# JacobYuan7/DIN-Group-Activity-Recognition-Benchmark

Measured on AMD Instinct MI355X. Metric: clips/sec (fwd+bwd), Volleyball DIN stage-2, BxTx12 actors, higher is better.
Workload: dtype bf16; 1 GPU; Volleyball stage-2 DIN, inv3, T=3, ST_kernel=(3,3), N=12, 720x1280, bf16; global_batch=32, clips_per_gpu=32, frames=3, parallelism=dp1, includes=fwd + cross-entropy + bwd + fused Adam (lr 0), launch_mode=eager launches, bn_mode=running statistics (set_bn_eval)

## Files before the change

din-group-activity-recognition-benchmark_amd/_lib.py:

```python
from __future__ import annotations

import ctypes as C
import os
import re
import subprocess
from typing import Dict, List

_HERE = os.path.dirname(os.path.abspath(__file__))
LIB_PATH = os.environ.get("DIN_LIB_PATH") or os.path.join(_HERE, "libdin_hip.so")
CSRC_DIR = os.path.join(_HERE, "csrc")
HEADER_PATH = os.path.join(os.path.dirname(_HERE), "include", "din_hip.h")

DIN_F32, DIN_BF16 = 0, 1
DIN_F32_BF16X3 = 2


def storage_dtype(dt: int) -> int:
    return DIN_F32 if dt == DIN_F32_BF16X3 else dt
ABI_VERSION = 9
CONV_BIAS, CONV_RELU, CONV_ACCUM, CONV_MASK = 1, 2, 4, 8


class DinError(RuntimeError):
    pass
# ... 34 lines not shown

SIGNATURES: Dict[str, tuple] = {
    "din_abi_version": (_I, []),
    "din_last_error_string": (C.c_char_p, []),
    "din_set_option": (_I, [C.c_char_p, C.c_char_p]),
    "din_get_option": (_I, [C.c_char_p, C.c_char_p, _I]),
    "din_build_arch": (C.c_char_p, []),
    "din_prep_images_f32": (_I, [_P, _P, _L, _P]),
    "din_prep_images_nhwc": (_I, [_P, _I, _P, _I, _I, _I, _I, _I, _P]),
    "din_conv_packed_elems": (_L, [_CD, _I]),
    "din_conv_pack_weights": (_I, [_CD, _P, _P, _P, _I, _P]),
    "din_conv_pack_desc": (_I, [_CD, _P, _P, _P, _I, C.POINTER(PackDesc)]),
    "din_conv_pack_multi": (_I, [_P, _P, _P, _I, _I, _P]),
    "din_conv_kernel_tile": (_I, [_CD, _I, C.POINTER(C.c_int32), C.POINTER(C.c_int32)]),
    "din_conv_kernel_variant": (_I, [_CD, _I, C.POINTER(C.c_int32)]),
    "din_conv_kernel_names": (_I, [_CD, _I, _I, _I, _I, C.c_char_p, _I]),
    "din_conv_workspace_bytes": (_L, [_CD, _I]),
    "din_conv_accepts_u8": (_I, [_P]),
    "din_conv_fwd": (_I, [_CD, _P, _P, _P, _P, _I, _P, _L, _P]),
    "din_conv_fwd2": (_I, [_CD, _P, _P, _P, _P, _P, _I, _I, _I, _I, _I, _P, _L, _P]),
    "din_conv_fwd2_kernel_names": (_I, [_CD, _I, _I, _I, _I, _I, C.c_char_p, _I]),
    "din_conv_dgrad": (_I, [_CD, _P, _P, _P, _P, _I, _I, _I, _P, _L, _P]),
    "din_conv1x1_dgrad_multi": (_I, [_I, C.POINTER(ConvSrc), _I, _I, _I, _I, _I, _I, _I, _P, _P, _I, _I, _I, _P]),
    "din_conv1x1_dgrad_multi_kernel_names": (_I, [_I, C.POINTER(ConvSrc), _I, _I, _I, _I, _I, _I, _I, _I, _I, _I, C.c_char_p, _I]),
    "din_conv_dgrad_x_fused": (_I, [_CD]),
    "din_conv_dgrad_x": (_I, [_CD, _P, _P, _P, _P, _I, _I, _I, C.POINTER(ConvSrc), _P, _L, _P]),
    "din_conv_dgrad_x_kernel_names": (_I, [_CD, C.POINTER(ConvSrc), _I, _I, _I, C.c_char_p, _I]),
    "din_conv1x1_wgrad_multi_workspace": (_L, [_I, C.POINTER(ConvWSrc), _I, _L, _I]),
    "din_conv1x1_wgrad_multi": (_I, [_I, C.POINTER(ConvWSrc), _I, _L, _I, _I, _I, _P, _I, _P, _L, _P]),
    "din_conv_wgrad_group_key": (_I, [_CD]),
    "din_conv_wgrad_group_workspace": (_L, [_I, C.POINTER(ConvWgradItem)]),
    "din_conv_wgrad_group": (_I, [_I, C.POINTER(ConvWgradItem), _P, _L, _P]),
    "din_conv_wgrad": (_I, [_CD, _P, _P, _P, _P, _P, _P, _P, _I, _P, _L, _P]),
    "din_colsum": (_I, [_P, _I, _L, _I, _I, _I, _P, _P]),
    "din_bn_fold": (_I, [_P, _P, _P, _P, _F, _P, _P, _I, _P]),
    "din_bn_fold_bwd": (_I, [_P, _P, _P, _P, _F, _P, _P, _I, _P]),
    "din_bn_fold_multi": (_I, [_P, _P, _I, _I, _F, _P, _P, _P]),
    "din_bn_fold_bwd_multi": (_I, [_P, _P, _I, _I, _F, _P, _P, _P, _P, _P]),
    "din_bn_stats": (_I, [_P, _I, _L, _I, _I, _I, _P, _P, _P]),
    "din_bn_parts": (_I, [_L]),
    "din_bn_workspace": (_L, [_L, _I]),
    "din_bn_reduce": (_I, [_P, _I, _I, _P]),
    "din_bn_finalize": (_I, [_P, _I, _L, _I, _P, _P, _F, _F, _P, _P, _P, _P, _P, _P, _P, _P]),
    "din_bn_apply": (_I, [_P, _I, _L, _I, _I, _I, _P, _P, _I, _P, _I, _I, _P]),
    "din_bn_bwd_stats": (_I, [_P, _I, _I, _P, _I, _I, _I, _L, _I, _P, _P, _P, _P]),
    "din_bn_bwd_apply": (_I, [_P, _I, _I, _P, _I, _I, _I, _L, _I, _P, _P, _P, _P, _P, _I, _I, _P, _P, _P]),
    "din_maxpool_fwd": (_I, [_PD, _P, _P, _P, _P]),
    "din_maxpool_bwd": (_I, [_PD, _P, _P, _P, _P, _I, _I, _P]),
    "din_avgpool_fwd": (_I, [_PD, _P, _P, _P, _I, _P]),
    "din_avgpool_bwd": (_I, [_PD, _P, _P, _P, _I, _P]),
    "din_bilinear_fwd": (_I, [_PD, _P, _P, _P]),
    "din_bilinear_bwd": (_I, [_PD, _P, _P, _P, _I, _P]),
    "din_pool_kernel_name": (_I, [_PD, _I, _I, _I, _I, C.c_char_p, _I]),
    "din_roi_align_fwd": (_I, [_P, _I, _I, _I, _I, _I, _I, _I, _I, _P, _P, _I, _I, _P, _I, _I, _P, _P]),
    "din_roi_align_bwd": (_I, [_P, _I, _I, _I, _I, _P, _P, _I, _I, _P, _P]),
    "din_roi_crop_grad_transpose": (_I, [_P, _I, _I, _I, _P, _P]),
    "din_roi_align_bwd_nhwc": (_I, [_P, _I, _I, _I, _I, _I, _I, _I, _I, _I, _P, _P, _I, _I, _P, _I, _I, _P, _I, _P]),
    "din_grad_cast_mask": (_I, [_P, _P, _P, _I, _L, _I, _I, _I, _I, _I, _I, _P]),
    "din_boxes_frame_index": (_I, [_P, _I, _I, _P]),
    "din_layernorm_fwd": (_I, [_P, _P, _P, _P, _F, _P, _P, _L, _L, _I, _F, _U64, _P, _P]),
    "din_layernorm_bwd": (_I, [_P, _P, _P, _P, _P, _P, _P, _P, _P, _L, _L, _I, _F, _U64, _P, _P]),
    "din_counter_add": (_I, [_P, _U64, _P]),
    "din_walk_fwd": (_I, [_P, _P, _I, _I, _I, _I, _I, _I, _I, _I, _I, _I, _P, _P, _P, _P, _P, _P, _P]),
    "din_walk_bwd": (_I, [_P, _P, _I, _P, _P, _I, _I, _I, _I, _I, _I, _I, _I, _I, _P, _P, _P, _P, _P, _P]),
    "din_head_fwd": (_I, [_P, _P, _P, _P, _I, _I, _I, _I, _I, _P, _P, _P]),
    "din_head_bwd": (_I, [_P, _P, _P, _P, _I, _I, _I, _I, _I, _P, _P, _P, _P]),
# ... 108 lines not shown
```

din-group-activity-recognition-benchmark_amd/csrc/conv_wgrad.h:

```cpp
#pragma once
#include "din_common.h"
#include <string>

namespace din_wgrad {

struct WgradK {
    const void* in; const void* g; float* partial; float* dbias;
    int NB, H, W, Cin, ldi, cioff;
    int OH, OW, Cout, ldo, cooff;
    int kh, kw, sh, sw, ph, pw, dh, dw;
    int cin_pad, kcols, kcols_pad, cout_pad;
    int M, n_co_tiles, n_k_tiles, slices, m_per_slice;
    int probe;
    const unsigned char* u8;
    int atomic;
    int pace_base;
    float* direct;
    int* pace;
};

constexpr int WGRAD_GROUP_MAX = 16;
struct WgradGroupK { WgradK k[WGRAD_GROUP_MAX]; int first[WGRAD_GROUP_MAX + 1]; int n; };

struct Wg1x1K {
// ... 7 lines not shown

__device__ __forceinline__ void lds_dma16(uint32_t lds_addr, __amdgpu_buffer_rsrc_t rs, int voff, int soff) {
    asm volatile("s_mov_b32 m0, %0\n\ts_nop 0\n\tbuffer_load_dwordx4 %1, %2, %3 offen lds"
                 :: "s"(lds_addr), "v"(voff), "s"(rs), "s"(soff) : "memory", "m0");
}

enum WgradFamily {
    WGRAD_F32,
    WGRAD_F32X3,
    WGRAD_BF16_TAIL,
    WGRAD_BF16,
    WGRAD_RING,
    WGRAD_PIPE,
    WGRAD_STEM,
    WGRAD_HALO
};
struct PipeInst { int bco, bk; bool wide; int wn; };
struct StemInst { int cpp, bn, st; bool u8; int nw, th, ring; };
struct HaloInst { int cpp, bnt, kh, kw, th; };
struct WgradChoice {
    WgradFamily family;
    int bco, bk;
    PipeInst pipe; StemInst stem; HaloInst halo;
    dim3 grid, block; size_t lds;
    bool bias_fused;
    int atomic;
    int group_key;
    int cin_pad, kcols, kcols_pad, cout_pad, n_co_tiles, n_k_tiles, slices, m_per_slice;
    int64_t ws_bytes;
};
WgradChoice plan_wgrad(const din_conv_desc* d, bool split = false);
void wgrad_tile_code(const WgradChoice& c, int32_t* bm, int32_t* bn);
void append_wgrad_names(const din_conv_desc* d, const WgradChoice& c, std::string& out);

int launch_wgrad_pipe(const WgradK& k, const PipeInst& inst, dim3 grid, dim3 block, size_t lds, hipStream_t st);
int launch_wgrad_pipe_group(const WgradGroupK& g, int bco, bool wide, hipStream_t st);
size_t wgrad_pipe_lds_bytes(int bco, int bk);
bool wgrad_halo_shape(int cin, int cout, int kh, int kw, HaloInst* inst);
size_t wgrad_halo_lds_bytes(const HaloInst& inst);
int launch_wgrad_halo(const WgradK& k, const HaloInst& inst, dim3 grid, dim3 block, size_t lds, hipStream_t st);
bool plan_wgrad_1x1_multi(int nsrc, const int* couts, int cin, Wg1x1K* k);
int launch_wgrad_1x1_multi(const Wg1x1K& k, int nwg, hipStream_t st);

}
```

din-group-activity-recognition-benchmark_amd/csrc/conv_wgrad.hip:

```cpp
#include "din_common.h"
#include "conv_wgrad.h"
#include "conv_shared.h"
#include <atomic>
#include <string>

using din_wgrad::WgradK;
using din_wgrad::WgradChoice;
using din_wgrad::lds_dma16;
using din_conv::check_desc;

namespace {

constexpr int WG_TILE = 128;

template <bool SPLIT>
__device__ __forceinline__ void conv_wgrad_f32_body(const WgradK& p) {
    constexpr int PK = 16;
    constexpr int RS = WG_TILE + 16;
    __shared__ float Gs[2][PK][RS];
    __shared__ float Xs[2][PK][RS];
    const int tid = threadIdx.x, lane = tid & 63, wid = tid >> 6;
    const int wm = wid >> 1, wn = wid & 1;
    int bid, slice_;
    xcd_block(bid, slice_);
// ... 1244 lines not shown
    } else if (v2) {
        w.family = WGRAD_BF16;
        w.lds = 2 * 64 * ((size_t)(w.bco * 2) + (WG_TILE * 2));
    } else {
        w.family = WGRAD_BF16_TAIL;
        w.lds = 2 * 2 * 32 * (WG_TILE * 2 + 32);
    }
    w.bias_fused = w.family != WGRAD_F32 && w.family != WGRAD_F32X3 && w.family != WGRAD_BF16_TAIL;
    return w;
}

void wgrad_tile_code(const WgradChoice& c, int32_t* bm, int32_t* bn) {
    switch (c.family) {
    case WGRAD_HALO: *bm = 3; *bn = c.bco; break;
    case WGRAD_STEM: *bm = 0; *bn = c.bco; break;
    case WGRAD_PIPE: *bm = c.bco; *bn = 2000 + c.bk; break;
    case WGRAD_RING: *bm = c.bco; *bn = 1000 + c.bk; break;
    default: *bm = c.bco; *bn = WG_TILE; break;
    }
}

void append_wgrad_names(const din_conv_desc* d, const WgradChoice& c, std::string& out) {
    out += wgrad_kernel_name(c); out += '\n';
    out += "conv_wgrad_reduce_kernel\n";
    if (!c.bias_fused) {
        const int unr = colsum_unroll(d->dtype, d->cout, d->ldo, d->cooff);
        const char* T = d->dtype == DIN_F32 ? "float" : "unsigned short";
        char s[64];
        if (unr) snprintf(s, sizeof s, "colsum_vec_kernel<%s, %d>\n", T, unr); else snprintf(s, sizeof s, "colsum_kernel<%s>\n", T);
        out += s;
    }
}

}

extern "C" {

int din_conv_wgrad(const din_conv_desc* d, const void* in, const void* dout, float* dw, float* dbias, const float* scale,
                   const float* w, float* wdot, int accumulate, void* workspace, int64_t workspace_bytes, void* stream) {
    const SplitDesc sd(d);
    if (int e = check_desc(d)) return e;
    DIN_REQUIRE(in && dout && dw, "conv_wgrad: null pointer");
    DIN_REQUIRE(!wdot || w, "conv_wgrad: wdot needs w");
    DIN_REQUIRE(!d->in_u8 || din_conv_accepts_u8(d), "conv_wgrad: in_u8 on a layer din_conv_accepts_u8() rejects");
    hipStream_t st = as_stream(stream);
    const bool prezeroed = (accumulate & 2) != 0;
    accumulate &= 1;
    const WgradChoice c = din_wgrad::plan_wgrad(d, sd.split);
    if (workspace_bytes < c.ws_bytes || !workspace)
        DIN_FAIL(DIN_E_WORKSPACE, "conv_wgrad: workspace %lld < %lld bytes", (long long)workspace_bytes, (long long)c.ws_bytes);
    DIN_REQUIRE(d->dtype == DIN_F32 || (d->ldo % 8 == 0 && d->cooff % 8 == 0), "conv_wgrad: bf16 dout stride/offset must be multiples of 8");
    WgradK k{};
    fill_wgrad_k(k, d, c, in, dout, workspace);
#ifdef DIN_EXPERIMENTS
    { const char* pv = DIN_OPT("DIN_WGRAD_PROBE"); k.probe = pv ? atoi(pv) : 0; }
#else
    k.probe = 0;
#endif
    if (dbias && c.bias_fused) {
        if (!prezeroed && hipMemsetAsync(dbias, 0, sizeof(float) * d->cout, st) != hipSuccess) DIN_FAIL(DIN_E_LAUNCH, "conv_wgrad: memset");
        k.dbias = dbias;
    }
    if (c.family == din_wgrad::WGRAD_PIPE) {
        k.atomic = c.atomic;
        if (c.atomic && hipMemsetAsync(k.partial, 0, sizeof(float) * (size_t)c.cout_pad * c.kcols_pad, st) != hipSuccess)
            DIN_FAIL(DIN_E_LAUNCH, "conv_wgrad: memset");
// ... 236 lines not shown
```

din-group-activity-recognition-benchmark_amd/nhwc.py:

```python
from __future__ import annotations

import ctypes as C
from dataclasses import dataclass, field
from typing import Dict, List, NamedTuple, Optional, Sequence, Tuple

import torch

from . import _lib as L


def _ptr(t: Optional[torch.Tensor]):
    return C.c_void_p(t.data_ptr()) if t is not None else None


def _stream():
    return C.c_void_p(torch.cuda.current_stream().cuda_stream)


def torch_dtype(dt: int):
    return torch.float32 if L.storage_dtype(dt) == L.DIN_F32 else torch.bfloat16


def din_dtype(t: torch.Tensor) -> int:
    if t.dtype == torch.float32:
        return L.DIN_F32
    if t.dtype == torch.bfloat16:
        return L.DIN_BF16
    raise L.DinError(f"unsupported storage dtype {t.dtype}")


def require_gpu(*tensors: torch.Tensor) -> None:
    for t in tensors:
        if t is None:
            continue
        if not t.is_cuda:
            raise L.DinError("din_amd ops run only on MI355X device tensors (no CPU fallback); got a CPU tensor")
        if not t.is_contiguous():
            raise L.DinError("din_amd ops need contiguous tensors")


import contextlib as _contextlib
LAUNCH_TIMER = None
TIMING_ACTIVE = lambda: LAUNCH_TIMER is not None


def _timed(kind, d, name=""):
    return LAUNCH_TIMER(kind, d, name) if LAUNCH_TIMER is not None else _contextlib.nullcontext()


GRAD_HOOK = None
GRAD_TAP = None
GRAD_BUFFER = None
GRAD_ASSIGN = None


def _dw_buffer(w: torch.Tensor) -> torch.Tensor:
    if GRAD_BUFFER is not None:
        buf = GRAD_BUFFER(w)
        if buf is not None:
            return buf
    return torch.empty_like(w)
FUSE_1X1_DGRAD = None
FUSE_FWD_SIBLINGS = None
FUSE_WGRAD_SIBLINGS = None
FUSE_WGRAD_1X1 = None
FUSE_DGRAD_X = None
GROUP_WGRAD = None
GROUP_WGRAD_MAX = 12
GROUP_WGRAD_MB = 768
_SWITCHES = {"FUSE_1X1_DGRAD": ("DIN_FUSE_1X1", True), "FUSE_FWD_SIBLINGS": ("DIN_FUSE_FWD", True), "FUSE_WGRAD_SIBLINGS": ("DIN_FUSE_WGRAD", True),
             "FUSE_WGRAD_1X1": ("DIN_FUSE_WGRAD_1X1", True), "FUSE_DGRAD_X": ("DIN_FUSE_DGRAD_X", True), "GROUP_WGRAD": ("DIN_GROUP_WGRAD", True), "WGRAD_SIDE_STREAM": ("DIN_WGRAD_STREAM", False)}


def switch(attr: str) -> bool:
    v = globals()[attr]
    if v is not None:
        return bool(v)
    name, default = _SWITCHES[attr]
    return L.host_flag(name, default)



_WS: Dict[Tuple[int, str], torch.Tensor] = {}


_SIDE: Dict[int, "torch.cuda.Stream"] = {}
WGRAD_SIDE_STREAM = None


def side_stream(device) -> "torch.cuda.Stream":
    key = device.index if device.index is not None else torch.cuda.current_device()
    if key not in _SIDE:
        _SIDE[key] = torch.cuda.Stream(device=device)
    return _SIDE[key]


def workspace(nbytes: int, device, tag: str = "") -> Tuple[Optional[torch.Tensor], int]:
    if nbytes <= 0:
        return None, 0
    key = (device.index if device.index is not None else torch.cuda.current_device(), tag)
    ws = _WS.get(key)
    if ws is None or ws.numel() < nbytes:
        ws = torch.empty(int(nbytes * 1.25) + 1024, dtype=torch.uint8, device=device)
        _WS[key] = ws
# ... 415 lines not shown
            aux.append((amax,))
        elif op.kind in ("avgpool", "bilinear"):
            d = _pool_desc(g, op, nb, dt)
            if op.kind == "avgpool":
                L.check(lib.din_avgpool_fwd(C.byref(d), _ptr(src), _ptr(dst), None, 0, st), "avgpool_fwd")
            else:
                L.check(lib.din_bilinear_fwd(C.byref(d), _ptr(src), _ptr(dst), st), "bilinear_fwd")
            aux.append(())
        else:
            raise L.DinError("unknown op " + op.kind)
    return bufs, aux


ViewKey = Tuple[int, int, int]


@dataclass
class BackwardPlan:
    offsets: List[int]
    bn_index: Dict[int, int]
    bn_train: bool
    side: bool
    u8: bool
    dgrad_groups: Dict[ViewKey, List[int]]
    member_of: Dict[int, ViewKey]
    x_host: Dict[int, int]
    siblings: Dict[int, Tuple[int, ...]]
    multi_w: Dict[ViewKey, Tuple[List[Tuple[int, ...]], int]]
    group_on: bool
    group_max: int
    group_bytes: int
    partitioned: set
    first_writer: Dict[int, int]


def _partitioned(readers: List[Tuple[int, int]], writers: Sequence[Tuple[int, int]]) -> bool:
    for (a0, ac), (b0, _bc) in zip(readers, readers[1:]):
        if b0 < a0 + ac:
            return False
    for lo, c in writers:
        hi = lo + c
        for c0, cc in readers:
            if c0 <= lo < c0 + cc:
                lo = min(hi, c0 + cc)
        if lo < hi:
            return False
    return True


def wgrad_queue_full(layers: int, held_bytes: int, max_layers: int, max_bytes: int) -> bool:
    return layers >= max_layers or held_bytes >= max_bytes


def plan_backward(g: Graph, nb: int, dt: int, bn_train: bool, side_ok: bool, u8: bool) -> BackwardPlan:
    lib = L.load()
    offsets, bn_index, pos = [], {}, 0
    readers: Dict[int, set] = {}
    writers: Dict[int, list] = {}
    first_writer: Dict[int, int] = {}
    for oi, op in enumerate(g.ops):
        if op.kind == "conv":
            offsets.append(pos)
            if op.bn:
                bn_index[oi] = len(bn_index)
            pos += 5 if op.bn else (2 if op.bias else 1)
        else:
# ... 29 lines not shown
        for grp in g.fwd_groups:
            mem = tuple(i for i in grp[1:] if g.ops[i].pooled is None)
            if len(mem) >= 2 and g.ops[mem[-1]].bn:
                siblings[mem[-1]] = mem
    multi_w: Dict[ViewKey, Tuple[List[Tuple[int, ...]], int]] = {}
    if switch("FUSE_WGRAD_1X1") and bn_index and not bn_train and not side and bf16:
        pair_of = {i: mem for mem in siblings.values() for i in mem}
        for key, members in groups.items():
            if not all(g.ops[i].bn for i in members):
                continue
            plan, seen = [], set()
            for i in members:
                if i in seen:
                    continue
                mem = pair_of.get(i, (i,))
                if not all(j in members for j in mem):
                    mem = (i,)
                plan.append(tuple(mem))
                seen.update(mem)
            probe = (L.ConvWSrc * len(plan))()
            for j, mem in enumerate(plan):
                o = g.ops[mem[0]]
                probe[j].cout = sum(g.ops[i].dst.c for i in mem)
                probe[j].ldo, probe[j].cooff = (o.dst.c, 0) if o.pooled is not None else (g.tensors[o.dst.tid].c, o.dst.coff)
            o0 = g.ops[members[0]]
            ts0 = g.tensors[o0.src.tid]
            need = lib.din_conv1x1_wgrad_multi_workspace(len(plan), probe, dt, nb * ts0.h * ts0.w, o0.src.c) if 2 <= len(plan) <= 4 else 0
            if need > 0:
                multi_w[key] = (plan, need)
    group_on = switch("GROUP_WGRAD") and bf16 and not side
    group_max = max(2, min(16, int(L.get_option("DIN_GROUP_WGRAD_MAX") or GROUP_WGRAD_MAX))) if group_on else 0
    group_bytes = int(L.get_option("DIN_GROUP_WGRAD_MB") or GROUP_WGRAD_MB) << 20 if group_on else 0
    return BackwardPlan(offsets, bn_index, bn_train, side, bool(u8), groups, member_of, x_host, siblings, multi_w, group_on, group_max,
                        group_bytes, partitioned, first_writer)


class _Pending(NamedTuple):
    oi: int
    gout: torch.Tensor
    w: torch.Tensor
    scale: Optional[torch.Tensor]
    ld: int
    coff: int
    pre: bool


class _Parked(NamedTuple):
    oi: int
    gout: torch.Tensor
    ld: int
    coff: int


class _Wgrad(NamedTuple):
    d: L.ConvDesc
    x: torch.Tensor
    gout: torch.Tensor
    dw: torch.Tensor
    dshift: Optional[torch.Tensor]
    scale: Optional[torch.Tensor]
    w: Optional[torch.Tensor]
    wdot: Optional[torch.Tensor]
    acc: int
    name: str
    outs: Tuple[Tuple[int, torch.Tensor], ...]


# ... 191 lines not shown
    def flush_group(self, key: ViewKey) -> None:
        items = self.pending[key]
        if not items:
            return
        g = self.g
        if key in self.plan.multi_w:
            self.flush_wgrad_multi(key, items)
        op0 = g.ops[items[0].oi]
        ts0 = g.tensors[op0.src.tid]
        gsrc, acc = self.grad_target(op0.src)
        srcs = (L.ConvSrc * len(items))()
        for j, it in enumerate(items):
            srcs[j].dout, srcs[j].wpk_t = it.gout.data_ptr(), self.pcache.wpt[it.oi].data_ptr()
            srcs[j].cout, srcs[j].ldo, srcs[j].cooff = g.ops[it.oi].dst.c, it.ld, it.coff
        d0 = _conv_desc(g, op0, self.nb, self.dt)
        d0.src_couts = tuple(g.ops[it.oi].dst.c for it in items)
        d0.cout = sum(d0.src_couts)
        with _timed("dgrad", d0, "+".join(g.ops[it.oi].name for it in items)):
            L.check(self.lib.din_conv1x1_dgrad_multi(len(items), srcs, self.dt, self.nb, ts0.h, ts0.w, op0.src.c, ts0.c, op0.src.coff, _ptr(gsrc),
                                                     self.mask_of(op0.src), ts0.c, op0.src.coff, self.dgrad_flags(op0.src, acc), self.st),
                    "conv1x1_dgrad_multi")
        self.pending[key] = []

    def dgrad_parked(self, host_oi: int) -> None:
        pk = self.parked.pop(host_oi)
        opj = self.g.ops[pk.oi]
        dj = _conv_desc(self.g, opj, self.nb, self.dt)
        dj.ldo, dj.cooff = pk.ld, pk.coff
        self.dgrad(pk.oi, dj, pk.gout)

    def dgrad(self, oi: int, d: L.ConvDesc, gout: torch.Tensor) -> None:
        op = self.g.ops[oi]
        ts = self.g.tensors[op.src.tid]
        gsrc, acc = self.grad_target(op.src)
        wpt = self.pcache.wpt[oi]
        flags = self.dgrad_flags(op.src, acc)
        ws, wsb = workspace(self.lib.din_conv_workspace_bytes(C.byref(d), 1), self.dev)
        pk = self.parked.pop(oi, None)
        if pk is not None:
            xs = L.ConvSrc()
            xs.dout, xs.wpk_t = pk.gout.data_ptr(), self.pcache.wpt[pk.oi].data_ptr()
            xs.cout, xs.ldo, xs.cooff = self.g.ops[pk.oi].dst.c, pk.ld, pk.coff
            with _timed("dgrad", d, op.name + "+" + self.g.ops[pk.oi].name):
                L.check(self.lib.din_conv_dgrad_x(C.byref(d), _ptr(gout), _ptr(wpt), _ptr(gsrc), self.mask_of(op.src), ts.c, op.src.coff, flags,
                                                  C.byref(xs), _ptr(ws), wsb, self.st), "conv_dgrad_x " + op.name)
        else:
            with _timed("dgrad", d, op.name):
                L.check(self.lib.din_conv_dgrad(C.byref(d), _ptr(gout), _ptr(wpt), _ptr(gsrc), self.mask_of(op.src), ts.c, op.src.coff, flags,
                                                _ptr(ws), wsb, self.st), "conv_dgrad " + op.name)

    def skip(self, oi: int) -> None:
        key = self.plan.member_of.get(oi)
        if key is not None:
            self.visited(key)
        if oi in self.parked:
            self.dgrad_parked(oi)

    def conv_step(self, oi: int, gout: torch.Tensor) -> _ConvStep:
        g, op = self.g, self.g.ops[oi]
        image = op.src.tid == g.input_tid
        d = _conv_desc(g, op, self.nb, self.dt, g.cin_image if image else op.src.c)
        if image and self.plan.u8:
            d.in_u8, d.ldi, d.cioff = 1, 8, 0
        return _ConvStep(d, gout, g.tensors[op.dst.tid].c, op.dst.coff)

    def bn_train_backward(self, oi: int, c: _ConvStep) -> None:
        g, lib, op, nb, dev, st = self.g, self.lib, self.g.ops[oi], self.nb, self.dev, self.st
        po, cout = self.plan.offsets[oi], op.dst.c
        _, raw, bmean, rstd = self.aux[oi]
        td = g.tensors[op.dst.tid]
        rows = nb * td.h * td.w
        sums = torch.empty(lib.din_bn_workspace(rows, cout) // 8, dtype=torch.float64, device=dev)
        L.check(lib.din_bn_bwd_stats(_ptr(c.gout), c.ld, c.coff, _ptr(raw), cout, 0, self.sdt, rows, cout, _ptr(bmean), _ptr(rstd),
                                     _ptr(sums), st), "bn_bwd_stats")
        dy = torch.empty((nb, td.h, td.w, cout), dtype=self.tdt, device=dev)
        dgb = torch.empty(2 * cout, dtype=torch.float32, device=dev)
        L.check(lib.din_bn_bwd_apply(_ptr(c.gout), c.ld, c.coff, _ptr(raw), cout, 0, self.sdt, rows, cout, _ptr(self.params[po + 1]), _ptr(bmean),
                                     _ptr(rstd), _ptr(sums), _ptr(dy), cout, 0, _ptr(dgb), _ptr(dgb[cout:]), st), "bn_bwd_apply")
        self.grads[po + 1], self.grads[po + 2] = dgb[:cout], dgb[cout:]
        c.gout, c.ld, c.coff = dy, cout, 0
        c.d.ldo, c.d.cooff = cout, 0
        if op.pooled is not None:
# ... 203 lines not shown
```

include/din_hip.h:

```cpp
#ifndef DIN_HIP_H
#define DIN_HIP_H

#include <stddef.h>
#include <stdint.h>

#ifdef __cplusplus
extern "C" {
#endif

#define DIN_ABI_VERSION 9

enum {
    DIN_F32 = 0, DIN_BF16 = 1,
    DIN_F32_BF16X3 = 2
};

enum {
    DIN_OK = 0,
    DIN_E_ARG = -1,
    DIN_E_LAUNCH = -2,
    DIN_E_WORKSPACE = -3,
    DIN_E_UNSUPPORTED = -4
};

// ... 37 lines not shown
                        int chunk_elems, void* stream);
int din_conv_fwd2(const din_conv_desc* d, const void* in, const void* wpk, const float* bias, void* out, void* out2, int ldo2, int cooff2,
                  int csplit, int craw, int flags, void* workspace, int64_t workspace_bytes, void* stream);
int din_conv_kernel_tile(const din_conv_desc* d, int which, int32_t* bm, int32_t* bn);
int din_conv_kernel_variant(const din_conv_desc* d, int which, int32_t* flags);
int din_conv_kernel_names(const din_conv_desc* d, int which, int flags, int ldm, int moff, char* buf, int buf_bytes);
int64_t din_conv_workspace_bytes(const din_conv_desc* d, int which );

int din_conv_accepts_u8(const din_conv_desc* d);

int din_conv_fwd(const din_conv_desc* d, const void* in, const void* wpk, const float* bias, void* out,
                 int flags, void* workspace, int64_t workspace_bytes, void* stream);
int din_conv_dgrad(const din_conv_desc* d, const void* dout, const void* wpk_t, void* din,
                   const void* mask, int ldm, int moff, int flags,
                   void* workspace, int64_t workspace_bytes, void* stream);
typedef struct din_conv_src {
    const void* dout;
    const void* wpk_t;
    int32_t cout, ldo, cooff;
} din_conv_src;
int din_conv1x1_dgrad_multi(int nsrc, const din_conv_src* srcs, int dtype, int nb, int h, int w, int cin, int ldi,
                            int cioff, void* din, const void* mask, int ldm, int moff, int flags, void* stream);
int din_conv_dgrad_x(const din_conv_desc* d, const void* dout, const void* wpk_t, void* din, const void* mask, int ldm, int moff, int flags,
                     const din_conv_src* x, void* workspace, int64_t workspace_bytes, void* stream);
int din_conv_dgrad_x_fused(const din_conv_desc* d);
int din_conv_fwd2_kernel_names(const din_conv_desc* d, int ldo2, int cooff2, int csplit, int craw, int flags, char* buf, int buf_bytes);
int din_conv1x1_dgrad_multi_kernel_names(int nsrc, const din_conv_src* srcs, int dtype, int nb, int h, int w, int cin, int ldi, int cioff,
                                         int ldm, int moff, int flags, char* buf, int buf_bytes);
int din_conv_dgrad_x_kernel_names(const din_conv_desc* d, const din_conv_src* x, int ldm, int moff, int flags, char* buf, int buf_bytes);
int din_conv_wgrad(const din_conv_desc* d, const void* in, const void* dout, float* dw, float* dbias,
                   const float* scale, const float* w, float* wdot, int accumulate,
                   void* workspace, int64_t workspace_bytes, void* stream);

typedef struct din_conv_wsrc {
    const void* dout;
    float* dw;
    float* dbias;
    const float* scale;
    const float* w;
    float* wdot;
    int32_t cout, ldo, cooff;
} din_conv_wsrc;
int64_t din_conv1x1_wgrad_multi_workspace(int nsrc, const din_conv_wsrc* srcs, int dtype, int64_t pixels, int cin);
int din_conv1x1_wgrad_multi(int nsrc, const din_conv_wsrc* srcs, int dtype, int64_t pixels, int cin, int ldi, int cioff, const void* in,
                            int accumulate, void* workspace, int64_t workspace_bytes, void* stream);

typedef struct din_conv_wgrad_item {
    din_conv_desc desc;
    const void* in;
    const void* dout;
    float* dw;
    float* dbias;
    const float* scale;
    const float* w;
    float* wdot;
    int32_t accumulate, reserved;
} din_conv_wgrad_item;
int din_conv_wgrad_group_key(const din_conv_desc* d);
int64_t din_conv_wgrad_group_workspace(int n, const din_conv_wgrad_item* items);
int din_conv_wgrad_group(int n, const din_conv_wgrad_item* items, void* workspace, int64_t workspace_bytes, void* stream);

int din_colsum(const void* g, int dtype, int64_t rows, int c, int ld, int coff, float* out, void* stream);

int din_bn_fold(const float* gamma, const float* beta, const float* mean, const float* var, float eps,
                float* scale, float* shift, int c, void* stream);
int din_bn_fold_bwd(const float* wdot, const float* dshift, const float* mean, const float* var, float eps,
// ... 154 lines not shown
```

Before: 631.4 clips/sec.

## Fuse second-conv data gradient with stem weight gradient in one kernel

Adds a fused kernel that computes the 3x3 32->32 data gradient into the stem's output, applies the ReLU mask, and immediately folds the result against the u8 input frames to accumulate the stem conv's weight gradient and bias gradient. The masked gradient stays in LDS instead of being written to global memory and re-read by a separate stem wgrad kernel. A partial-sum reduce kernel then finishes dw. The planner enables this by default when the graph pattern matches (bf16, u8 input, frozen BN). The cost is a complex hand-tuned kernel with hard-coded wait counts, higher LDS use, and atomics for the bias.

```diff
diff --git a/din-group-activity-recognition-benchmark_amd/_lib.py b/din-group-activity-recognition-benchmark_amd/_lib.py
--- a/din-group-activity-recognition-benchmark_amd/_lib.py
+++ b/din-group-activity-recognition-benchmark_amd/_lib.py
@@ -90,6 +90,9 @@
     "din_conv_wgrad_group_workspace": (_L, [_I, C.POINTER(ConvWgradItem)]),
     "din_conv_wgrad_group": (_I, [_I, C.POINTER(ConvWgradItem), _P, _L, _P]),
     "din_conv_wgrad": (_I, [_CD, _P, _P, _P, _P, _P, _P, _P, _I, _P, _L, _P]),
+    "din_conv_stem_fold_ok": (_I, [_CD, _I, _I, _I, _CD, C.POINTER(C.c_int64)]),
+    "din_conv_stem_fold": (_I, [_CD, _P, _P, _P, _I, _I, _I, _CD, _P, _P, _P, _P, _P, _P, _I, _P, _L, _P]),
+    "din_conv_stem_fold_kernel_names": (_I, [_CD, _I, _I, _I, _CD, C.c_char_p, _I]),
     "din_colsum": (_I, [_P, _I, _L, _I, _I, _I, _P, _P]),
     "din_bn_fold": (_I, [_P, _P, _P, _P, _F, _P, _P, _I, _P]),
     "din_bn_fold_bwd": (_I, [_P, _P, _P, _P, _F, _P, _P, _I, _P]),
diff --git a/din-group-activity-recognition-benchmark_amd/csrc/conv_stem_fold.hip b/din-group-activity-recognition-benchmark_amd/csrc/conv_stem_fold.hip
--- /dev/null
+++ b/din-group-activity-recognition-benchmark_amd/csrc/conv_stem_fold.hip
@@ -0,0 +1,387 @@
+#include "din_common.h"
+#include "conv_wgrad.h"
+#include "conv_gather.h"
+#include "conv_shared.h"
+#include <stdlib.h>
+#include <string.h>
+
+using din_wgrad::lds_dma16;
+using din_gather::ConvK;
+using din_gather::SmallVariant;
+
+namespace {
+
+constexpr int FOLD_GRID = 512;
+constexpr int FOLD_CIN_PAD = 4, FOLD_KCOLS_PAD = 48, FOLD_COUT_PAD = 32;
+
+__device__ __forceinline__ u32x2 lds_tr_read(uint32_t byte_addr) {
+    u32x2 r;
+    asm volatile("ds_read_b64_tr_b16 %0, %1" : "=v"(r) : "v"(byte_addr) : "memory");
+    return r;
+}
+
+struct FoldK {
+    ConvK c;
+    const unsigned char* u8;
+    int IH, IW, iph, ipw;
+    int icout;
+    float* partial;
+    float* dbias;
+};
+
+template <int CPP, int BN, int NBUF, int NW>
+__global__ __launch_bounds__(64 * NW, 2) void conv_small_fold_kernel(FoldK a) {
+    static_assert(CPP == 4 && BN == 32 && NBUF == 2 && NW == 4, "written for the 32 -> 32 data gradient on four waves");
+#if defined(__HIP_DEVICE_COMPILE__)
+    typedef bf16_t T;
+    const ConvK& p = a.c;
+    constexpr int NTHREADS = 64 * NW;
+    constexpr int KH = 3, KW = 3, TH = 8, TW = 32, NPX = TH * TW;
+    constexpr int TI = BN / 16, TJ = 16 / NW, NTAPS = KH * KW;
+    constexpr int HWW = TW - 1 + KW, HWH = TH - 1 + KH, HPX = HWW * HWH, HC = HPX * CPP;
+    constexpr int WBYTES = NTAPS * BN * CPP * 16;
+    constexpr int HBYTES = (HC * 16 + 1023) / 1024 * 1024;
+    constexpr int NSLOT = HBYTES / 1024, NTR = (NSLOT + NW - 1) / NW;
+    constexpr int SPITCH = BN * 2;
+    static_assert(NPX * SPITCH <= HBYTES, "staging does not fit the halo buffer");
+    constexpr int CPR = BN / 8, NIT = NPX * CPR / NTHREADS;
+    constexpr int IWW = (TW - 1) * 2 + KW, IHH = (TH - 1) * 2 + KH, IPX = IWW * IHH, IPITCH = 81;
+    constexpr int NSLOT_I = (IPX + 63) / 64, NTR_I = (NSLOT_I + NW - 1) / NW;
+    constexpr int IBYTES = (IHH * IPITCH * 8 + 511) / 512 * 512;
+    constexpr unsigned OOB = 0x80000000u;
+    extern __shared__ __attribute__((aligned(16))) unsigned char smem_raw[];
+    const int tid = threadIdx.x, lane = tid & 63, wid = tid >> 6;
+    u32x4* Wl = reinterpret_cast<u32x4*>(smem_raw);
+    unsigned char* Xl = smem_raw + WBYTES + NBUF * HBYTES;
+    bf16_t* u8lut = reinterpret_cast<bf16_t*>(Xl + IBYTES);
+    auto swz = [](int row) { return (row >> 1) & 3; };
+    auto swzG = [](int t) { return ((t >> 2) & 1) * 2; };
+
+    {
+        const u32x4* __restrict__ wp = reinterpret_cast<const u32x4*>(p.w);
+        for (int id = tid; id < NTAPS * BN * CPP; id += NTHREADS) {
+            const int row = id / CPP, slot = id - row * CPP;
+            const int tap = row / BN, co = row - tap * BN;
+            Wl[id] = wp[(int64_t)co * p.wld + tap * CPP + (slot ^ swz(co))];
+        }
+    }
+    u8_lut_init(u8lut, tid);
+    int rel[NTR];
+    short hyv[NTR], hxv[NTR];
+#pragma unroll
+    for (int i = 0; i < NTR; ++i) {
+        const int id = (wid + NW * i) * 64 + lane;
+        const int hp = id / CPP, slot = id - hp * CPP;
+        const int cc = slot ^ swz(hp);
+        const int hy = hp / HWW, hx = hp - hy * HWW;
+        rel[i] = id < HC ? (hy * p.W + hx) * p.ldi * 2 + cc * 16 : -1;
+        hyv[i] = (short)hy; hxv[i] = (short)hx;
+    }
+    int iin[NTR_I];
+    short iyv[NTR_I], ixv[NTR_I];
+#pragma unroll
+    for (int i = 0; i < NTR_I; ++i) {
+        const int id = (wid + NW * i) * 64 + lane;
+        const int iy = id / IWW, ix = id - iy * IWW;
+        iin[i] = id < IPX ? 0 : -1;
+        iyv[i] = (short)iy; ixv[i] = (short)ix;
+    }
+    const int hy0 = p.by + (p.cy < 0 ? (KH - 1) * p.cy : 0), hx0 = p.bx + (p.cx < 0 ? (KW - 1) * p.cx : 0);
+    const int tiles_x = (p.OW + TW - 1) / TW, tiles_y = (p.OH + TH - 1) / TH;
+    const int tiles_img = tiles_x * tiles_y, ntiles = tiles_img * p.NB;
+    const long long img_bytes = (long long)p.H * p.W * p.ldi * 2ll, mimg_bytes = (long long)p.OH * p.OW * p.ldm * 2ll;
+    const uint32_t lds_base = (uint32_t)(uintptr_t)smem_raw;
+    const uint32_t ldsH0 = __builtin_amdgcn_readfirstlane(lds_base + (uint32_t)WBYTES + (uint32_t)(wid * 1024));
+
+    auto issue_halo = [&](int buf, int tile) {
+        const int n = tile / tiles_img;
+        const int tr = tile - n * tiles_img;
+        const int ty = tr / tiles_x, tx = tr - ty * tiles_x;
+        const int gy0 = ty * TH + hy0, gx0 = tx * TW + hx0;
+        __amdgpu_buffer_rsrc_t rs = __builtin_amdgcn_make_buffer_rsrc(
+            const_cast<char*>(reinterpret_cast<const char*>(p.in)) + (long long)n * img_bytes, 0, (int)img_bytes, 0x00020000);
+        const int base = (gy0 * p.W + gx0) * p.ldi * 2 + p.cioff * 2;
+        const uint32_t dst = ldsH0 + (uint32_t)(buf * HBYTES);
+#pragma unroll
+        for (int i = 0; i < NTR; ++i) {
+            if (wid + NW * i < NSLOT) {
+                const int gy = gy0 + hyv[i], gx = gx0 + hxv[i];
+                const bool ok = rel[i] >= 0 && gy >= 0 && gy < p.H && gx >= 0 && gx < p.W;
+                lds_dma16(dst + (uint32_t)(i * 1024 * NW), rs, ok ? base + rel[i] : (int)OOB, 0);
+            }
+        }
+    };
+    U8Halo<NTR_I> u8h;
+    auto u8_load = [&](int tile) {
+        const int n = tile / tiles_img;
+        const int tr = tile - n * tiles_img;
+        const int ty = tr / tiles_x, tx = tr - ty * tiles_x;
+        u8h.template load<NSLOT_I>(a.u8, n, a.IH, a.IW, ty * TH * 2 - a.iph, tx * TW * 2 - a.ipw, wid, iyv, ixv, iin);
+    };
+    auto u8_store = [&]() {
+#pragma unroll
+        for (int i = 0; i < NTR_I; ++i) {
+            if (wid + NW * i < NSLOT_I && iin[i] >= 0) {
+                u32x2 v = {0u, 0u};
+                if ((u8h.valid >> i) & 1u) {
+                    v[0] = (uint32_t)u8lut[u8h.r[i]] | ((uint32_t)u8lut[u8h.g[i]] << 16);
+                    v[1] = (uint32_t)u8lut[u8h.b[i]];
+                }
+                *reinterpret_cast<u32x2*>(Xl + ((int)iyv[i] * IPITCH + (int)ixv[i]) * 8) = v;
+            }
+        }
+    };
+
+    const int frow0 = lane & 15, g40 = lane >> 4;
+    const int xq = g40 * 4 + (frow0 >> 2), quad = frow0 & 3;
+    const bool col_wave = wid < 3;
+    const int ftap = min(4 * wid + quad, NTAPS - 1);
+    const uint32_t xoff = (uint32_t)(((ftap / KW) * IPITCH + (ftap % KW) + xq * 2) * 8);
+    const uint32_t goff = (uint32_t)(xq * SPITCH + (((quad >> 1) ^ swzG(xq)) * 16) + (quad & 1) * 8);
+    const uint32_t Xb = lds_base + (uint32_t)(WBYTES + NBUF * HBYTES);
+    const u32x4 ones = {0x3f803f80u, 0x3f803f80u, 0x3f803f80u, 0x3f803f80u};
+    f32x4 wacc[TI];
+#pragma unroll
+    for (int i = 0; i < TI; ++i) wacc[i] = f32x4{0.f, 0.f, 0.f, 0.f};
+
+    auto fold = [&](int buf) {
+        const uint32_t Gb = lds_base + (uint32_t)(WBYTES + buf * HBYTES);
+        u32x4 gf[2][TI], xf[2];
+        auto load_frags = [&](int ks, u32x4 (&gfr)[TI], u32x4& xfr) {
+#pragma unroll
+            for (int i = 0; i < TI; ++i) {
+                u32x2 rr[2];
+#pragma unroll
+                for (int rd = 0; rd < 2; ++rd)
+                    rr[rd] = lds_tr_read(Gb + (uint32_t)((ks * 32 + rd * 16) * SPITCH) + (goff ^ (uint32_t)(i * 32)));
+                gfr[i] = u32x4{rr[0][0], rr[0][1], rr[1][0], rr[1][1]};
+            }
+            if (col_wave) {
+                u32x2 rr[2];
+#pragma unroll
+                for (int rd = 0; rd < 2; ++rd) rr[rd] = lds_tr_read(Xb + (uint32_t)((ks * 2 * IPITCH + rd * 32) * 8) + xoff);
+                xfr = u32x4{rr[0][0], rr[0][1], rr[1][0], rr[1][1]};
+            } else xfr = ones;
+        };
+        load_frags(0, gf[0], xf[0]);
+        asm volatile("s_waitcnt lgkmcnt(0)" ::: "memory");
+        __builtin_amdgcn_sched_barrier(0);
+#pragma unroll
+        for (int ks = 0; ks < TH; ++ks) {
+            if (ks + 1 < TH) load_frags(ks + 1, gf[(ks + 1) & 1], xf[(ks + 1) & 1]);
+#pragma unroll
+            for (int i = 0; i < TI; ++i)
+                wacc[i] = __builtin_amdgcn_mfma_f32_16x16x32_bf16(__builtin_bit_cast(bf16x8, gf[ks & 1][i]), __builtin_bit_cast(bf16x8, xf[ks & 1]), wacc[i], 0, 0, 0);
+            asm volatile("s_waitcnt lgkmcnt(0)" ::: "memory");
+            __builtin_amdgcn_sched_barrier(0);
+        }
+    };
+
+    u32x4 mkN[NIT];
+#pragma unroll
+    for (int it = 0; it < NIT; ++it) mkN[it] = u32x4{0u, 0u, 0u, 0u};
+    constexpr int YOUNGER = NTR - 1 + 3 * NTR_I;
+    static_assert(NSLOT % NW != 0 && NSLOT / NW == NTR - 1 && YOUNGER < 64, "the hand-counted waits assume 22 halo slots on four waves");
+    auto mask_load = [&](int tile, u32x4 (&mk)[NIT]) {
+        const int n = tile / tiles_img;
+        const int trm = tile - n * tiles_img;
+        const int ty = trm / tiles_x, tx = trm - ty * tiles_x;
+        __amdgpu_buffer_rsrc_t rsM = __builtin_amdgcn_make_buffer_rsrc(
+            const_cast<char*>(reinterpret_cast<const char*>(p.mask)) + (long long)n * mimg_bytes, 0, (int)mimg_bytes, 0x00020000);
+#pragma unroll
+        for (int it = 0; it < NIT; ++it) {
+            const int idx = it * NTHREADS + tid;
+            const int t = idx / CPR, c = idx - t * CPR;
+            const int gy = ty * TH + (t >> 5), gx = tx * TW + (t & 31);
+            const bool ok = gy < p.OH && gx < p.OW;
+            const int off = ok ? ((gy * p.OW + gx) * p.ldm + p.moff + c * 8) * 2 : (int)OOB;
+            asm volatile("buffer_load_dwordx4 %0, %1, %2, 0 offen" : "+v"(mk[it]) : "v"(off), "s"(rsM) : "memory");
+        }
+    };
+    int cur = 0;
+    int tile = xcd_remap((int)blockIdx.x, (int)gridDim.x);
+    if (tile < ntiles) { issue_halo(0, tile); u8_load(tile); mask_load(tile, mkN); }
+    __syncthreads();
+    const int ysgn = p.cy > 0 ? 1 : -1, xsgn = p.cx > 0 ? 1 : -1;
+    const int yb = p.cy > 0 ? 0 : KH - 1, xb = p.cx > 0 ? 0 : KW - 1;
+    for (; tile < ntiles; tile += gridDim.x) {
+        asm volatile("s_waitcnt vmcnt(%0)" :: "n"(NIT) : "memory");
+        u8h.landed();
+        __builtin_amdgcn_s_barrier();
+        asm volatile("" ::: "memory");
+        u8_store();
+        const bool have_next = tile + (int)gridDim.x < ntiles;
+        if (have_next) { issue_halo(cur ^ 1, tile + gridDim.x); u8_load(tile + gridDim.x); }
+        const u32x4* Hl = reinterpret_cast<const u32x4*>(smem_raw + WBYTES + cur * HBYTES);
+        int frow = frow0, g4 = g40, tidv = tid;
+        asm volatile("" : "+v"(frow), "+v"(g4), "+v"(tidv));
+        f32x4 acc[TI][TJ];
+#pragma unroll
+        for (int i = 0; i < TI; ++i)
+#pragma unroll
+            for (int j = 0; j < TJ; ++j) acc[i][j] = f32x4{0.f, 0.f, 0.f, 0.f};
+        u32x4 wf[2][TI], xf[2][TJ];
+        auto load_tap = [&](int tap, u32x4 (&wfr)[TI], u32x4 (&xfr)[TJ]) {
+            const int r = tap / KW, s2 = tap - r * KW;
+            const int dy = yb + ysgn * r, dx = xb + xsgn * s2;
+#pragma unroll
+            for (int i = 0; i < TI; ++i) {
+                const int co = i * 16 + frow;
+                wfr[i] = Wl[(tap * BN + co) * CPP + (g4 ^ swz(co))];
+            }
+#pragma unroll
+            for (int j = 0; j < TJ; ++j) {
+                const int q = wid * TJ + j;
+                const int hp = ((q >> 1) + dy) * HWW + (q & 1) * 16 + frow + dx;
+                xfr[j] = Hl[hp * CPP + (g4 ^ swz(hp))];
+            }
+        };
+        load_tap(0, wf[0], xf[0]);
+#pragma unroll
+        for (int tap = 0; tap < NTAPS; ++tap) {
+            if (tap + 1 < NTAPS) load_tap(tap + 1, wf[(tap + 1) & 1], xf[(tap + 1) & 1]);
+#pragma unroll
+            for (int i = 0; i < TI; ++i)
+#pragma unroll
+                for (int j = 0; j < TJ; ++j) Mma<T>::run(wf[tap & 1][i], xf[tap & 1][j], acc[i][j]);
+            __builtin_amdgcn_sched_barrier(0);
+        }
+        __syncthreads();
+        unsigned char* stg = smem_raw + WBYTES + cur * HBYTES;
+#pragma unroll
+        for (int i = 0; i < TI; ++i)
+#pragma unroll
+            for (int j = 0; j < TJ; ++j) {
+                const int t = (wid * TJ + j) * 16 + frow;
+                const f32x4 v = acc[i][j];
+                *reinterpret_cast<u32x2*>(stg + t * SPITCH + (((i * 2 + (g4 >> 1)) ^ swzG(t)) * 16) + (g4 & 1) * 8) =
+                    u32x2{pack_bf16x2(v[0], v[1]), pack_bf16x2(v[2], v[3])};
+            }
+        __syncthreads();
+        if (have_next) asm volatile("s_waitcnt vmcnt(%0)" :: "n"(YOUNGER) : "memory");
+        else asm volatile("s_waitcnt vmcnt(0)" ::: "memory");
+#pragma unroll
+        for (int it = 0; it < NIT; ++it) asm volatile("" : "+v"(mkN[it]));
+#pragma unroll
+        for (int it = 0; it < NIT; ++it) {
+            const int idx = it * NTHREADS + tidv;
+            const int t = idx / CPR, c = idx - t * CPR;
+            u32x4* slot = reinterpret_cast<u32x4*>(stg + t * SPITCH + ((c ^ swzG(t)) * 16));
+            u32x4 v = *slot;
+            const u32x4 mk = mkN[it];
+#pragma unroll
+            for (int e = 0; e < 4; ++e) {
+                float lo = __uint_as_float(v[e] << 16), hi = __uint_as_float(v[e] & 0xffff0000u);
+                if (!(__uint_as_float(mk[e] << 16) > 0.f)) lo = 0.f;
+                if (!(__uint_as_float(mk[e] & 0xffff0000u) > 0.f)) hi = 0.f;
+                v[e] = pack_bf16x2(lo, hi);
+            }
+            *slot = v;
+        }
+        if (have_next) mask_load(tile + gridDim.x, mkN);
+        __syncthreads();
+        fold(cur);
+        cur ^= 1;
+    }
+    const int frow = frow0, g4 = g40;
+    if (col_wave) {
+        float* dst = a.partial + (int64_t)blockIdx.x * (FOLD_COUT_PAD * FOLD_KCOLS_PAD);
+#pragma unroll
+        for (int i = 0; i < TI; ++i) {
+            const int co = i * 16 + g4 * 4;
+#pragma unroll
+            for (int e = 0; e < 4; ++e) dst[(co + e) * FOLD_KCOLS_PAD + wid * 16 + frow] = wacc[i][e];
+        }
+    } else if (a.dbias != nullptr && frow == 0) {
+#pragma unroll
+        for (int i = 0; i < TI; ++i) {
+            const int co = i * 16 + g4 * 4;
+#pragma unroll
+            for (int e = 0; e < 4; ++e) if (co + e < a.icout) atomicAdd(a.dbias + co + e, wacc[i][e]);
+        }
+    }
+#endif
+}
+
+const char* const FOLD_KERNEL_NAME = "conv_small_fold_kernel<4,32,2,4>";
+constexpr size_t FOLD_LDS = 9 * 32 * 4 * 16 + 2 * 22528 + 11264 + 512;
+
+bool fold_plan(const din_conv_desc* d2, int ldm, int moff, int flags, const din_conv_desc* d1, FoldK* out) {
+    if (!d2 || !d1 || din_conv::check_desc(d2) != DIN_OK || din_conv::check_desc(d1) != DIN_OK) return false;
+    if (opt_int(DIN_OPT("DIN_STEM_FOLD"), 1) == 0) return false;
+    if (d2->dtype != DIN_BF16 || d1->dtype != DIN_BF16 || flags != DIN_CONV_MASK) return false;
+    if (!d1->in_u8 || !din_conv_accepts_u8(d1) || d1->cin > 8 || d1->cout != 32) return false;
+    if (d2->in_u8 || d2->kh != 3 || d2->kw != 3 || d2->sh != 1 || d2->sw != 1 || d2->dh != 1 || d2->dw != 1 || d2->cin != 32 || d2->cout != 32) return false;
+    if (d2->nb != d1->nb || d2->h != d1->oh || d2->w != d1->ow) return false;
+    if (d2->ldo % 8 != 0 || d2->cooff % 8 != 0 || d2->ldo < d2->cooff + 32 || ldm < moff + 32) return false;
+    if ((int64_t)d2->nb * d2->oh * d2->ow < 256 * 1024) return false;
+    FoldK f{};
+    ConvK& k = f.c;
+    const PackGeom bank = pack_geom(d2, 1);
+    k.NB = d2->nb; k.kh = 3; k.kw = 3;
+    k.H = d2->oh; k.W = d2->ow; k.Cin = d2->cout; k.ldi = d2->ldo; k.cioff = d2->cooff;
+    k.OH = d2->h; k.OW = d2->w; k.Cout = d2->cin; k.ldo = d2->ldi; k.cooff = d2->cioff;
+    k.ay = 1; k.by = d2->ph; k.cy = -1; k.divy = 1;
+    k.ax = 1; k.bx = d2->pw; k.cx = -1; k.divx = 1;
+    k.M = d2->nb * d2->h * d2->w;
+    k.in_bytes = (long long)d2->nb * d2->oh * d2->ow * d2->ldo * 2;
+    k.w_bytes = (long long)bank.rows_pad * bank.kelems * 2;
+    k.cpt = bank.cpt; k.Q = 9 * bank.cpt; k.nk = bank.nk; k.wld = bank.nk * KC; k.splitk = 1; k.ks_per_split = bank.nk; k.n_co_tiles = 1;
+    k.flags = flags; k.ldm = ldm; k.moff = moff;
+    SmallVariant s{};
+    if (!din_gather::conv_small_variant(k, DIN_BF16, s)) return false;
+    if (s.cpt != 4 || s.bn != 32 || s.nbuf != 2 || s.waves != 4 || !s.epi || s.image) return false;
+    f.IH = d1->h; f.IW = d1->w; f.iph = d1->ph; f.ipw = d1->pw; f.icout = d1->cout;
+    if (out) *out = f;
+    return true;
+}
+
+}
+
+extern "C" {
+
+int din_conv_stem_fold_ok(const din_conv_desc* d2a, int ldm, int moff, int flags, const din_conv_desc* d1a, int64_t* workspace_bytes) {
+    const bool ok = fold_plan(d2a, ldm, moff, flags, d1a, nullptr);
+    if (workspace_bytes) *workspace_bytes = ok ? (int64_t)FOLD_GRID * FOLD_COUT_PAD * FOLD_KCOLS_PAD * 4 : 0;
+    return ok ? 1 : 0;
+}
+
+int din_conv_stem_fold_kernel_names(const din_conv_desc* d2a, int ldm, int moff, int flags, const din_conv_desc* d1a, char* buf, int buf_bytes) {
+    DIN_REQUIRE(buf_bytes >= 0 && (buf || buf_bytes == 0), "conv_stem_fold_kernel_names: bad argument");
+    DIN_REQUIRE(fold_plan(d2a, ldm, moff, flags, d1a, nullptr), "conv_stem_fold_kernel_names: not a pair din_conv_stem_fold_ok() accepts");
+    const std::string names = std::string(FOLD_KERNEL_NAME) + "\nconv_wgrad_reduce_kernel\n";
+    if (buf_bytes > 0) {
+        const size_t n = names.size() < (size_t)buf_bytes - 1 ? names.size() : (size_t)buf_bytes - 1;
+        memcpy(buf, names.data(), n);
+        buf[n] = 0;
+    }
+    return (int)names.size() + 1;
+}
+
+int din_conv_stem_fold(const din_conv_desc* d2a, const void* dout, const void* wpk_t, const void* mask, int ldm, int moff, int flags,
+                       const din_conv_desc* d1a, const void* frames, float* dw, float* dbias, const float* scale, const float* w, float* wdot,
+                       int accumulate, void* workspace, int64_t workspace_bytes, void* stream) {
+    FoldK f{};
+    DIN_REQUIRE(fold_plan(d2a, ldm, moff, flags, d1a, &f), "conv_stem_fold: not a pair din_conv_stem_fold_ok() accepts");
+    DIN_REQUIRE(dout && wpk_t && mask && frames && dw, "conv_stem_fold: null pointer");
+    DIN_REQUIRE(!wdot || w, "conv_stem_fold: wdot needs w");
+    const int64_t need = (int64_t)FOLD_GRID * FOLD_COUT_PAD * FOLD_KCOLS_PAD * 4;
+    if (workspace_bytes < need || !workspace)
+        DIN_FAIL(DIN_E_WORKSPACE, "conv_stem_fold: workspace %lld < %lld bytes", (long long)workspace_bytes, (long long)need);
+    hipStream_t st = as_stream(stream);
+    const bool prezeroed = (accumulate & 2) != 0;
+    f.c.in = dout; f.c.w = wpk_t; f.c.mask = mask;
+    f.u8 = reinterpret_cast<const unsigned char*>(frames);
+    f.partial = reinterpret_cast<float*>(workspace);
+    f.dbias = dbias;
+    if (dbias && !prezeroed && hipMemsetAsync(dbias, 0, sizeof(float) * d1a->cout, st) != hipSuccess) DIN_FAIL(DIN_E_LAUNCH, "conv_stem_fold: memset");
+    auto kern = conv_small_fold_kernel<4, 32, 2, 4>;
+    raise_lds_limit(kern, FOLD_LDS);
+    hipLaunchKernelGGL(kern, dim3(FOLD_GRID), dim3(256), FOLD_LDS, st, f);
+    DIN_CHECK_LAUNCH("conv_stem_fold");
+    if (wdot && !prezeroed && hipMemsetAsync(wdot, 0, sizeof(float) * d1a->cout, st) != hipSuccess) DIN_FAIL(DIN_E_LAUNCH, "conv_stem_fold: memset");
+    return din_wgrad::launch_wgrad_reduce(f.partial, dw, scale, w, wdot, d1a->cout, d1a->cin, 3, 3, FOLD_CIN_PAD, FOLD_COUT_PAD, FOLD_KCOLS_PAD,
+                                          FOLD_GRID, accumulate & 1, st);
+}
+
+}
diff --git a/din-group-activity-recognition-benchmark_amd/csrc/conv_wgrad.h b/din-group-activity-recognition-benchmark_amd/csrc/conv_wgrad.h
--- a/din-group-activity-recognition-benchmark_amd/csrc/conv_wgrad.h
+++ b/din-group-activity-recognition-benchmark_amd/csrc/conv_wgrad.h
@@ -63,6 +63,8 @@
 WgradChoice plan_wgrad(const din_conv_desc* d, bool split = false);
 void wgrad_tile_code(const WgradChoice& c, int32_t* bm, int32_t* bn);
 void append_wgrad_names(const din_conv_desc* d, const WgradChoice& c, std::string& out);
+int launch_wgrad_reduce(const float* partial, float* dw, const float* scale, const float* w, float* wdot, int cout, int cin, int kh, int kw,
+                        int cin_pad, int cout_pad, int kcols_pad, int slices, int accumulate, hipStream_t st);
 
 int launch_wgrad_pipe(const WgradK& k, const PipeInst& inst, dim3 grid, dim3 block, size_t lds, hipStream_t st);
 int launch_wgrad_pipe_group(const WgradGroupK& g, int bco, bool wide, hipStream_t st);
diff --git a/din-group-activity-recognition-benchmark_amd/csrc/conv_wgrad.hip b/din-group-activity-recognition-benchmark_amd/csrc/conv_wgrad.hip
--- a/din-group-activity-recognition-benchmark_amd/csrc/conv_wgrad.hip
+++ b/din-group-activity-recognition-benchmark_amd/csrc/conv_wgrad.hip
@@ -1300,6 +1300,16 @@
     }
 }
 
+int launch_wgrad_reduce(const float* partial, float* dw, const float* scale, const float* w, float* wdot, int cout, int cin, int kh, int kw,
+                        int cin_pad, int cout_pad, int kcols_pad, int slices, int accumulate, hipStream_t st) {
+    const dim3 rgrid(cout, (kh * kw * cin_pad + 255) / 256);
+    const int nsg = slices >= 64 ? 16 : slices >= 8 ? 4 : 1;
+    hipLaunchKernelGGL(conv_wgrad_reduce_kernel, rgrid, dim3(64, nsg), 0, st, partial, dw, scale, w, wdot, cout, cin, kh, kw, cin_pad, cout_pad,
+                       kcols_pad, slices, accumulate);
+    DIN_CHECK_LAUNCH("conv_wgrad_reduce");
+    return DIN_OK;
+}
+
 }
 
 extern "C" {
diff --git a/din-group-activity-recognition-benchmark_amd/nhwc.py b/din-group-activity-recognition-benchmark_amd/nhwc.py
--- a/din-group-activity-recognition-benchmark_amd/nhwc.py
+++ b/din-group-activity-recognition-benchmark_amd/nhwc.py
@@ -50,6 +50,7 @@
 
 GRAD_HOOK = None
 GRAD_TAP = None
+GRAD_TAP_MAPS = None
 GRAD_BUFFER = None
 GRAD_ASSIGN = None
 
@@ -65,11 +66,13 @@
 FUSE_WGRAD_SIBLINGS = None
 FUSE_WGRAD_1X1 = None
 FUSE_DGRAD_X = None
+FUSE_STEM_FOLD = None
 GROUP_WGRAD = None
 GROUP_WGRAD_MAX = 12
 GROUP_WGRAD_MB = 768
 _SWITCHES = {"FUSE_1X1_DGRAD": ("DIN_FUSE_1X1", True), "FUSE_FWD_SIBLINGS": ("DIN_FUSE_FWD", True), "FUSE_WGRAD_SIBLINGS": ("DIN_FUSE_WGRAD", True),
-             "FUSE_WGRAD_1X1": ("DIN_FUSE_WGRAD_1X1", True), "FUSE_DGRAD_X": ("DIN_FUSE_DGRAD_X", True), "GROUP_WGRAD": ("DIN_GROUP_WGRAD", True), "WGRAD_SIDE_STREAM": ("DIN_WGRAD_STREAM", False)}
+             "FUSE_WGRAD_1X1": ("DIN_FUSE_WGRAD_1X1", True), "FUSE_DGRAD_X": ("DIN_FUSE_DGRAD_X", True), "FUSE_STEM_FOLD": ("DIN_FUSE_STEM_FOLD", True),
+             "GROUP_WGRAD": ("DIN_GROUP_WGRAD", True), "WGRAD_SIDE_STREAM": ("DIN_WGRAD_STREAM", False)}
 
 
 def switch(attr: str) -> bool:
@@ -551,6 +554,7 @@
     group_bytes: int
     partitioned: set
     first_writer: Dict[int, int]
+    fold: Optional[Tuple[int, int]] = None
 
 
 def _partitioned(readers: List[Tuple[int, int]], writers: Sequence[Tuple[int, int]]) -> bool:
@@ -646,7 +650,36 @@
     group_max = max(2, min(16, int(L.get_option("DIN_GROUP_WGRAD_MAX") or GROUP_WGRAD_MAX))) if group_on else 0
     group_bytes = int(L.get_option("DIN_GROUP_WGRAD_MB") or GROUP_WGRAD_MB) << 20 if group_on else 0
     return BackwardPlan(offsets, bn_index, bn_train, side, bool(u8), groups, member_of, x_host, siblings, multi_w, group_on, group_max,
-                        group_bytes, partitioned, first_writer)
+                        group_bytes, partitioned, first_writer, _plan_stem_fold(g, nb, dt, bn_train, side, bool(u8), member_of, x_host))
+
+
+def _plan_stem_fold(g: Graph, nb: int, dt: int, bn_train: bool, side: bool, u8: bool, member_of, x_host) -> Optional[Tuple[int, int]]:
+    if not (switch("FUSE_STEM_FOLD") and u8 and dt == L.DIN_BF16 and not bn_train and not side):
+        return None
+    first = [oi for oi, op in enumerate(g.ops) if op.src.tid == g.input_tid]
+    if len(first) != 1:
+        return None
+    o1 = first[0]
+    op1 = g.ops[o1]
+    tid = op1.dst.tid
+    if GRAD_TAP is not None and GRAD_TAP_MAPS is not None and (GRAD_TAP_MAPS is True or tid in GRAD_TAP_MAPS):
+        return None
+    above = [oi for oi, op in enumerate(g.ops) if op.src.tid == tid]
+    producers = [oi for oi, op in enumerate(g.ops) if op.dst.tid == tid]
+    ts = g.tensors[tid]
+    if len(above) != 1 or producers != [o1] or tid in g.output_tids or not ts.relu_masked:
+        return None
+    o2 = above[0]
+    op2 = g.ops[o2]
+    if not (op1.kind == "conv" and op1.bn and op1.pooled is None and (op1.dst.coff, op1.dst.c) == (0, ts.c)):
+        return None
+    if not (op2.kind == "conv" and op2.pooled is None and o2 not in member_of and o2 not in x_host and o2 not in x_host.values()):
+        return None
+    d1 = _conv_desc(g, op1, nb, dt, g.cin_image)
+    d1.in_u8, d1.ldi, d1.cioff = 1, 8, 0
+    d2 = _conv_desc(g, op2, nb, dt, op2.src.c)
+    ok = L.load().din_conv_stem_fold_ok(C.byref(d2), ts.c, op2.src.coff, L.CONV_MASK, C.byref(d1), None)
+    return (o1, o2) if ok == 1 else None
 
 
 class _Pending(NamedTuple):
@@ -904,6 +937,9 @@
     def dgrad(self, oi: int, d: L.ConvDesc, gout: torch.Tensor) -> None:
         op = self.g.ops[oi]
         ts = self.g.tensors[op.src.tid]
+        if self.plan.fold is not None and oi == self.plan.fold[1] and op.src.tid not in self.gbufs:
+            self.stem_fold(oi, d, gout)
+            return
         gsrc, acc = self.grad_target(op.src)
         wpt = self.pcache.wpt[oi]
         flags = self.dgrad_flags(op.src, acc)
@@ -920,6 +956,28 @@
             with _timed("dgrad", d, op.name):
                 L.check(self.lib.din_conv_dgrad(C.byref(d), _ptr(gout), _ptr(wpt), _ptr(gsrc), self.mask_of(op.src), ts.c, op.src.coff, flags,
                                                 _ptr(ws), wsb, self.st), "conv_dgrad " + op.name)
+
+    def stem_fold(self, oi: int, d: L.ConvDesc, gout: torch.Tensor) -> None:
+        g, lib = self.g, self.lib
+        o1 = self.plan.fold[0]
+        op, op1 = g.ops[oi], g.ops[o1]
+        ts = g.tensors[op.src.tid]
+        d1 = _conv_desc(g, op1, self.nb, self.dt, g.cin_image)
+        d1.in_u8, d1.ldi, d1.cioff = 1, 8, 0
+        po = self.plan.offsets[o1]
+        w, scale = self.params[po], self.aux[o1][0]
+        dw = _dw_buffer(w)
+        o0, o1b = self.bn_range(o1)
+        self.bn_touched = True
+        need = C.c_int64(0)
+        if lib.din_conv_stem_fold_ok(C.byref(d), ts.c, op.src.coff, L.CONV_MASK, C.byref(d1), C.byref(need)) != 1:
+            raise L.DinError(f"graph_backward: the stem fold planned for {op.name} + {op1.name} is not served at launch time")
+        ws, wsb = workspace(need.value, self.dev)
+        with _timed("dgrad", d, op.name + "+wgrad:" + op1.name):
+            L.check(lib.din_conv_stem_fold(C.byref(d), _ptr(gout), _ptr(self.pcache.wpt[oi]), self.mask_of(op.src), ts.c, op.src.coff, L.CONV_MASK,
+                                           C.byref(d1), _ptr(self.bufs[g.input_tid]), _ptr(dw), _ptr(self.bn_dshift[o0:o1b]), _ptr(scale), _ptr(w),
+                                           _ptr(self.bn_wdot[o0:o1b]), 2, _ptr(ws), wsb, self.st), "conv_stem_fold " + op.name)
+        self.report(o1, dw)
 
     def skip(self, oi: int) -> None:
         key = self.plan.member_of.get(oi)
diff --git a/include/din_hip.h b/include/din_hip.h
--- a/include/din_hip.h
+++ b/include/din_hip.h
@@ -93,6 +93,12 @@
                    const float* scale, const float* w, float* wdot, int accumulate,
                    void* workspace, int64_t workspace_bytes, void* stream);
 
+int din_conv_stem_fold_ok(const din_conv_desc* d2a, int ldm, int moff, int flags, const din_conv_desc* d1a, int64_t* workspace_bytes);
+int din_conv_stem_fold(const din_conv_desc* d2a, const void* dout, const void* wpk_t, const void* mask, int ldm, int moff, int flags,
+                       const din_conv_desc* d1a, const void* frames, float* dw, float* dbias, const float* scale, const float* w, float* wdot,
+                       int accumulate, void* workspace, int64_t workspace_bytes, void* stream);
+int din_conv_stem_fold_kernel_names(const din_conv_desc* d2a, int ldm, int moff, int flags, const din_conv_desc* d1a, char* buf, int buf_bytes);
+
 typedef struct din_conv_wsrc {
     const void* dout;
     float* dw;
```

Result: no change. 634.0 clips/sec (median of 6 runs) (+0.4%).
